# vfrantc/Bayesian-Enhancement-Model

Hardware: AMD Instinct MI355X
Metric: images/sec (whole node) CG_UNet N=8 Bayesian eval @256x256 (higher is better)
Workload: dtype f32

## Files before the change

### bayesian-enhancement-model_amd/csrc/conv.hip

```cpp
#include "bem_common.h"

namespace {

constexpr int RB = 4;

__device__ __forceinline__ void dw_block(const float* __restrict__ plane, int H, int W, int y0, int x0, bool vec,
                                         const float* __restrict__ w9, float (&acc)[RB][4]) {
    float wk[9];
#pragma unroll
    for (int i = 0; i < 9; ++i) wk[i] = w9[i];
#pragma unroll
    for (int ry = -1; ry <= RB; ++ry) {
        const int yy = y0 + ry;
        if (yy < 0 || yy >= H) continue;
        const float* r = plane + (int64_t)yy * W;
        float v[6];
        v[0] = x0 > 0 ? r[x0 - 1] : 0.f;
        if (vec) {
            const float4 c = *reinterpret_cast<const float4*>(r + x0);
            v[1] = c.x; v[2] = c.y; v[3] = c.z; v[4] = c.w;
        } else {
#pragma unroll
            for (int i = 0; i < 4; ++i) v[1 + i] = (x0 + i < W) ? r[x0 + i] : 0.f;
        }
        v[5] = (x0 + 4 < W) ? r[x0 + 4] : 0.f;
#pragma unroll
        for (int oy = 0; oy < RB; ++oy) {
            const int dy = ry - oy;
            if (dy < -1 || dy > 1) continue;
            const float w0 = wk[(dy + 1) * 3], w1 = wk[(dy + 1) * 3 + 1], w2 = wk[(dy + 1) * 3 + 2];
#pragma unroll
            for (int j = 0; j < 4; ++j) acc[oy][j] = fmaf(w0, v[j], fmaf(w1, v[j + 1], fmaf(w2, v[j + 2], acc[oy][j])));
        }
    }
}

__global__ __launch_bounds__(256) void dwconv3x3_kernel(const float* __restrict__ x, const float* __restrict__ w,
                                                        int64_t w_bs, const float* __restrict__ bias, int64_t b_bs,
                                                        float* __restrict__ out, int Cout, int H, int W, int mode) {
    const int W4 = (W + 3) >> 2, HB = (H + RB - 1) / RB;
    const int i = blockIdx.x * blockDim.x + threadIdx.x;
    if (i >= HB * W4) return;
    const int yb = i / W4, y0 = yb * RB, x0 = (i - yb * W4) * 4;
    const int c = blockIdx.y, b = blockIdx.z;
    const int Cin = (mode == 2) ? 2 * Cout : Cout;
    const int64_t HW = (int64_t)H * W;
    const bool vec = (W & 3) == 0;
    const float* wb = w + (int64_t)b * w_bs;
    const float* bb = bias ? bias + (int64_t)b * b_bs : nullptr;
    float a0[RB][4];
#pragma unroll
    for (int r = 0; r < RB; ++r)
#pragma unroll
        for (int j = 0; j < 4; ++j) a0[r][j] = 0.f;
    const float* pl = x + ((int64_t)b * Cin + c) * HW;
    dw_block(pl, H, W, y0, x0, vec, wb + (int64_t)c * 9, a0);
    const float b0 = bb ? bb[c] : 0.f;
    float a1[RB][4];
    float b1 = 0.f;
    if (mode == 2) {
#pragma unroll
        for (int r = 0; r < RB; ++r)
#pragma unroll
            for (int j = 0; j < 4; ++j) a1[r][j] = 0.f;
        dw_block(x + ((int64_t)b * Cin + c + Cout) * HW, H, W, y0, x0, vec, wb + (int64_t)(c + Cout) * 9, a1);
        b1 = bb ? bb[c + Cout] : 0.f;
    }
#pragma unroll
    for (int r = 0; r < RB; ++r) {
        const int y = y0 + r;
        if (y >= H) break;
        float o[4];
#pragma unroll
        for (int j = 0; j < 4; ++j) {
            const float v = a0[r][j] + b0;
            if (mode == 2) o[j] = bem_gelu(v) * (a1[r][j] + b1);
            else if (mode == 1) o[j] = bem_silu(v);
            else if (mode == 3) o[j] = ((x0 + j < W) ? pl[(int64_t)y * W + x0 + j] : 0.f) + fmaxf(v, 0.f);
            else o[j] = v;
        }
        float* op = out + ((int64_t)b * Cout + c) * HW + (int64_t)y * W + x0;
        if (vec) {
            *reinterpret_cast<float4*>(op) = make_float4(o[0], o[1], o[2], o[3]);
        } else {
#pragma unroll
            for (int j = 0; j < 4; ++j)
                if (x0 + j < W) op[j] = o[j];
        }
    }
}

__device__ __forceinline__ float dpp_from_prev_lane(float v) {
    return __builtin_bit_cast(float, __builtin_amdgcn_update_dpp(0, __builtin_bit_cast(int, v), 0x138, 0xf, 0xf, false));
}
__device__ __forceinline__ float dpp_from_next_lane(float v) {
    return __builtin_bit_cast(float, __builtin_amdgcn_update_dpp(0, __builtin_bit_cast(int, v), 0x130, 0xf, 0xf, false));
}

template <bool DPPHALO>
__device__ __forceinline__ void dw_block_fast(const float* __restrict__ plane, int H, int W, int y0, int x0,
                                              const float* __restrict__ w9, float (&acc)[RB][4]) {
    float4 c[RB + 2];
    float hl[RB + 2], hr[RB + 2];
#pragma unroll
    for (int ry = -1; ry <= RB; ++ry) {
        const int yy = min(max(y0 + ry, 0), H - 1);
        const float* r = plane + (int64_t)yy * W;
        c[ry + 1] = *reinterpret_cast<const float4*>(r + x0);
        if (!DPPHALO) {
            hl[ry + 1] = r[max(x0 - 1, 0)];
            hr[ry + 1] = r[min(x0 + 4, W - 1)];
        }
    }
    float wk[9];
#pragma unroll
    for (int i = 0; i < 9; ++i) wk[i] = w9[i];
    const float mt = y0 > 0 ? 1.f : 0.f, mb = y0 + RB < H ? 1.f : 0.f;
    const float ml = x0 > 0 ? 1.f : 0.f, mr = x0 + 4 < W ? 1.f : 0.f;
#pragma unroll
    for (int ry = -1; ry <= RB; ++ry) {
        float4 q = c[ry + 1];
        if (ry == -1) { q.x *= mt; q.y *= mt; q.z *= mt; q.w *= mt; }
        if (ry == RB) { q.x *= mb; q.y *= mb; q.z *= mb; q.w *= mb; }
        const float v[6] = {(DPPHALO ? dpp_from_prev_lane(q.w) : hl[ry + 1] * ((ry == -1) ? mt : (ry == RB) ? mb : 1.f)) * ml, q.x, q.y, q.z, q.w,
                            (DPPHALO ? dpp_from_next_lane(q.x) : hr[ry + 1] * ((ry == -1) ? mt : (ry == RB) ? mb : 1.f)) * mr};
#pragma unroll
        for (int oy = 0; oy < RB; ++oy) {
            const int dy = ry - oy;
            if (dy < -1 || dy > 1) continue;
            const float w0 = wk[(dy + 1) * 3], w1 = wk[(dy + 1) * 3 + 1], w2 = wk[(dy + 1) * 3 + 2];
#pragma unroll
            for (int j = 0; j < 4; ++j) acc[oy][j] = fmaf(w0, v[j], fmaf(w1, v[j + 1], fmaf(w2, v[j + 2], acc[oy][j])));
        }
    }
}

template <int MODE, bool DPPHALO>
__global__ __launch_bounds__(256) void dwconv3x3_fast_kernel(const float* __restrict__ x, const float* __restrict__ w,
                                                             int64_t w_bs, const float* __restrict__ bias, int64_t b_bs,
                                                             float* __restrict__ out, int Cout, int H, int W) {
    const int W4 = W >> 2, HB = H / RB;
    const int i = blockIdx.x * blockDim.x + threadIdx.x;
    if (i >= HB * W4) return;
    const int yb = i / W4, y0 = yb * RB, x0 = (i - yb * W4) * 4;
    const int c = blockIdx.y, b = blockIdx.z;
    const int Cin = (MODE == 2) ? 2 * Cout : Cout;
    const int64_t HW = (int64_t)H * W;
    const float* wb = w + (int64_t)b * w_bs;
    const float* bb = bias ? bias + (int64_t)b * b_bs : wb;
    const float bm = bias ? 1.f : 0.f;
    const float b0 = bb[bias ? c : 0] * bm;
    const float b1 = (MODE == 2) ? bb[bias ? c + Cout : 0] * bm : 0.f;
    const float* pl = x + ((int64_t)b * Cin + c) * HW;
    float a0[RB][4], a1[RB][4];
#pragma unroll
    for (int r = 0; r < RB; ++r)
#pragma unroll
        for (int j = 0; j < 4; ++j) a0[r][j] = a1[r][j] = 0.f;
    dw_block_fast<DPPHALO>(pl, H, W, y0, x0, wb + (int64_t)c * 9, a0);
    if (MODE == 2) dw_block_fast<DPPHALO>(x + ((int64_t)b * Cin + c + Cout) * HW, H, W, y0, x0, wb + (int64_t)(c + Cout) * 9, a1);
    float4 self[RB];
    if (MODE == 3) {
#pragma unroll
        for (int r = 0; r < RB; ++r) self[r] = *reinterpret_cast<const float4*>(pl + (int64_t)(y0 + r) * W + x0);
    }
#pragma unroll
    for (int r = 0; r < RB; ++r) {
        float o[4];
        const float sv[4] = {MODE == 3 ? self[r].x : 0.f, MODE == 3 ? self[r].y : 0.f, MODE == 3 ? self[r].z : 0.f, MODE == 3 ? self[r].w : 0.f};
#pragma unroll
        for (int j = 0; j < 4; ++j) {
            const float v = a0[r][j] + b0;
            if (MODE == 2) o[j] = bem_gelu_fast(v) * (a1[r][j] + b1);
            else if (MODE == 1) o[j] = bem_silu(v);
            else if (MODE == 3) o[j] = sv[j] + fmaxf(v, 0.f);
            else o[j] = v;
        }
        *reinterpret_cast<float4*>(out + ((int64_t)b * Cout + c) * HW + (int64_t)(y0 + r) * W + x0) = make_float4(o[0], o[1], o[2], o[3]);
    }
}

constexpr int TH = 8, TW = 32, COB = 16, CIB = 8;

template <int KH, int KW, int S>
__global__ __launch_bounds__(256) void conv2d_kernel(const float* __restrict__ x, int64_t x_bs,
                                                     const float* __restrict__ w, const float* __restrict__ bias,
                                                     const float* __restrict__ res1, const float* __restrict__ res2,
                                                     float* __restrict__ out, int Cin, int H, int W, int Cout,
                                                     int Ho, int Wo, int pad, int relu, int tilesX, int res1_rep) {
    constexpr int PH = (TH - 1) * S + KH, PW = (TW - 1) * S + KW;
    constexpr int PWP = PW + 1;
    __shared__ float patch[CIB][PH][PWP];
    __shared__ __attribute__((aligned(16))) float wl[CIB][KH * KW][COB];
    const int tile = blockIdx.x;
    const int ty0 = (tile / tilesX) * TH, tx0 = (tile % tilesX) * TW;
    const int co0 = blockIdx.y * COB;
    const int b = blockIdx.z;
    const int tx = threadIdx.x & 31, ty = threadIdx.x >> 5;
    const int oy = ty0 + ty, ox = tx0 + tx;
    const int iy0 = ty0 * S - pad, ix0 = tx0 * S - pad;
    const float* xb = x + (int64_t)b * x_bs;
    float acc[COB];
#pragma unroll
    for (int i = 0; i < COB; ++i) acc[i] = 0.f;
    for (int ci0 = 0; ci0 < Cin; ci0 += CIB) {
        __syncthreads();
        for (int i = threadIdx.x; i < CIB * PH * PW; i += 256) {
            const int cc = i / (PH * PW), rem = i - cc * (PH * PW);
            const int py = rem / PW, px = rem - py * PW;
            const int ci = ci0 + cc, iy = iy0 + py, ix = ix0 + px;
            float v = 0.f;
            if (ci < Cin && iy >= 0 && iy < H && ix >= 0 && ix < W) v = xb[((int64_t)ci * H + iy) * W + ix];
            patch[cc][py][px] = v;
        }
        for (int i = threadIdx.x; i < CIB * KH * KW * COB; i += 256) {
            const int o = i % COB, t = (i / COB) % (KH * KW), cc = i / (COB * KH * KW);
            const int ci = ci0 + cc, co = co0 + o;
            wl[cc][t][o] = (ci < Cin && co < Cout) ? w[(((int64_t)co * Cin + ci) * KH * KW) + t] : 0.f;
        }
        __syncthreads();
#pragma unroll 2
        for (int cc = 0; cc < CIB; ++cc) {
#pragma unroll
            for (int ky = 0; ky < KH; ++ky) {
#pragma unroll
                for (int kx = 0; kx < KW; ++kx) {
                    const float v = patch[cc][ty * S + ky][tx * S + kx];
                    const float4* wq = reinterpret_cast<const float4*>(&wl[cc][ky * KW + kx][0]);
#pragma unroll
                    for (int q = 0; q < COB / 4; ++q) {
                        const float4 ww = wq[q];
                        acc[4 * q] = fmaf(ww.x, v, acc[4 * q]);
                        acc[4 * q + 1] = fmaf(ww.y, v, acc[4 * q + 1]);
                        acc[4 * q + 2] = fmaf(ww.z, v, acc[4 * q + 2]);
                        acc[4 * q + 3] = fmaf(ww.w, v, acc[4 * q + 3]);
                    }
                }
            }
        }
    }
    if (oy >= Ho || ox >= Wo) return;
#pragma unroll
    for (int o = 0; o < COB; ++o) {
        const int co = co0 + o;
        if (co >= Cout) break;
        float v = acc[o] + (bias ? bias[co] : 0.f);
        if (relu) v = fmaxf(v, 0.f);
        const int64_t idx = (((int64_t)b * Cout + co) * Ho + oy) * Wo + ox;
        if (res1) v += res1[(((int64_t)(b / res1_rep) * Cout + co) * Ho + oy) * Wo + ox];
        if (res2) v += res2[idx];
        out[idx] = v;
    }
}


typedef float f32x16 __attribute__((ext_vector_type(16)));

template <int KH, int KW, int PH, int PWP>
__device__ __forceinline__ constexpr int patch_off(int k) {
    return (k / (KH * KW)) * PH * PWP + ((k % (KH * KW)) / KW) * PWP + (k % (KH * KW)) % KW;
}

template <int MTW>
__device__ __forceinline__ void conv_mfma_epilogue(f32x16 (&acc)[MTW][2], const float* __restrict__ Wp, const float* __restrict__ bias,
                                                   const float* __restrict__ res1, const float* __restrict__ res2,
                                                   float* __restrict__ out, int b, int b1, int Cout, int Ho, int Wo, int ty0, int tx0,
                                                   int wave, int half, int j, int relu) {
    const int ox = tx0 + j, oxc = min(ox, Wo - 1);
    const float* bp = bias ? bias : Wp;
    const float* p1 = res1 ? res1 : Wp;
    const float* p2 = res2 ? res2 : Wp;
    const float bmk = bias ? 1.f : 0.f, m1 = res1 ? 1.f : 0.f, m2 = res2 ? 1.f : 0.f;
    const int64_t k0 = bias ? -1 : 0, k1 = res1 ? -1 : 0, k2 = res2 ? -1 : 0;
    const float lo = relu ? 0.f : -3.402823466e38f;
    const int64_t b1off = (int64_t)(b1 - b) * Cout * Ho * Wo;
#pragma unroll
    for (int t = 0; t < 2; ++t) {
        const int oy = ty0 + 2 * wave + t, oyc = min(oy, Ho - 1);
        const bool pix = oy < Ho && ox < Wo;
#pragma unroll
        for (int m = 0; m < MTW; ++m) {
            constexpr int RG = 8;
#pragma unroll
            for (int r0 = 0; r0 < 16; r0 += RG) {
                float r1[RG], r2[RG], bv[RG];
#pragma unroll
                for (int q = 0; q < RG; ++q) {
                    const int r = r0 + q;
                    const int co = min(m * 32 + (r & 3) + 8 * (r >> 2) + 4 * half, Cout - 1);
                    const int64_t idx = (((int64_t)b * Cout + co) * Ho + oyc) * Wo + oxc;
                    bv[q] = bp[co & k0] * bmk;
                    r1[q] = p1[(idx + b1off) & k1] * m1;
                    r2[q] = p2[idx & k2] * m2;
                }
#pragma unroll
                for (int q = 0; q < RG; ++q) {
                    const int r = r0 + q;
                    const int co = m * 32 + (r & 3) + 8 * (r >> 2) + 4 * half;
                    if (pix && co < Cout)
                        out[(((int64_t)b * Cout + co) * Ho + oy) * Wo + ox] = fmaxf(acc[m][t][r] + bv[q], lo) + r1[q] + r2[q];
                }
            }
        }
    }
}

template <int KH, int KW, int S, int MTW>
__global__ __launch_bounds__(256, MTW == 1 ? 4 : MTW == 2 ? 3 : MTW == 3 ? 2 : 1) void conv2d_mfma_kernel(const float* __restrict__ x, int64_t x_bs,
                                                          const float* __restrict__ Wp, const float* __restrict__ bias,
                                                          const float* __restrict__ res1, const float* __restrict__ res2,
                                                          float* __restrict__ out, int Cin, int H, int W, int Cout,
                                                          int Ho, int Wo, int pad, int relu, int tilesX, int KS, int res1_rep) {
    constexpr int KK = KH * KW;
    constexpr int KC = CIB * KK;
    constexpr int PH = (TH - 1) * S + KH, PW = (TW - 1) * S + KW, PWP = PW + 1;
    __shared__ float patch[CIB * PH * PWP];
    const int lane = threadIdx.x & 63, wave = threadIdx.x >> 6, half = lane >> 5, j = lane & 31;
    const int tile = blockIdx.x, b = blockIdx.y;
    const int ty0 = (tile / tilesX) * TH, tx0 = (tile % tilesX) * TW;
    const int iy0 = ty0 * S - pad, ix0 = tx0 * S - pad;
    const float* xb = x + (int64_t)b * x_bs;
    f32x16 acc[MTW][2];
#pragma unroll
    for (int m = 0; m < MTW; ++m)
#pragma unroll
        for (int t = 0; t < 2; ++t)
#pragma unroll
            for (int r = 0; r < 16; ++r) acc[m][t][r] = 0.f;
    const float* wl = Wp + lane;
    const int64_t mts = (int64_t)KS * 64;
    const int rowoff0 = (2 * wave) * S * PWP + j * S, rowoff1 = rowoff0 + S * PWP;
// ... 37 lines not shown
            for (int u = 0; u < PB; ++u)
                an[m][u] = wl[m * mts + (int64_t)min(sg0 + u, KS - 1) * 64] * ((sg0 + u < KS) ? 1.f : 0.f);
        for (int s0 = 0; s0 < NS; s0 += PB) {
            float ac[MTW][PB];
#pragma unroll
            for (int m = 0; m < MTW; ++m)
#pragma unroll
                for (int u = 0; u < PB; ++u) {
                    ac[m][u] = an[m][u];
                    const int sn = sg0 + s0 + PB + u;
                    an[m][u] = wl[m * mts + (int64_t)min(sn, KS - 1) * 64] * ((s0 + PB + u < NS && sn < KS) ? 1.f : 0.f);
                }
#pragma unroll
            for (int u = 0; u < PB; ++u) {
                const int k = 2 * (s0 + u) + half, kc = k / KK, kt = k - kc * KK;
                const int o = kc * PH * PWP + (kt / KW) * PWP + (kt % KW);
                const float v0 = patch[o + rowoff0], v1 = patch[o + rowoff1];
#pragma unroll
                for (int m = 0; m < MTW; ++m) {
                    acc[m][0] = __builtin_amdgcn_mfma_f32_32x32x2f32(ac[m][u], v0, acc[m][0], 0, 0, 0);
                    acc[m][1] = __builtin_amdgcn_mfma_f32_32x32x2f32(ac[m][u], v1, acc[m][1], 0, 0, 0);
                }
            }
        }
    }
    conv_mfma_epilogue<MTW>(acc, Wp, bias, res1, res2, out, b, b / res1_rep, Cout, Ho, Wo, ty0, tx0, wave, half, j, relu);
}

template <int KH, int KW, int S, int MTW>
__global__ __launch_bounds__(256, MTW == 1 ? 3 : 2) void conv2d_mfma_pipe_kernel(const float* __restrict__ x, int64_t x_bs,
                                                               const float* __restrict__ Wp, const float* __restrict__ bias,
                                                               const float* __restrict__ res1, const float* __restrict__ res2,
                                                               float* __restrict__ out, int Cin, int H, int W, int Cout,
                                                               int Ho, int Wo, int pad, int relu, int tilesX, int KS, int res1_rep) {
    constexpr int KK = KH * KW;
    constexpr int KC = CIB * KK;
    constexpr int NS = KC / 2;
    constexpr int PH = (TH - 1) * S + KH, PW = (TW - 1) * S + KW, PWP = PW + 1;
    constexpr int PSZ = CIB * PH * PWP;
    constexpr int TOT = CIB * PH * PW;
    constexpr int NU = (TOT + 255) / 256;
    constexpr int WSZ = NS * 64;
    static_assert(WSZ % 256 == 0, "weight slice must split evenly over the workgroup");
    constexpr int NWU = WSZ / 256;
    __shared__ float patch[2][PSZ + 1];
    __shared__ float wsm[2][MTW][WSZ];
    const int lane = threadIdx.x & 63, wave = threadIdx.x >> 6, half = lane >> 5, j = lane & 31;
    const int tile = blockIdx.x, b = blockIdx.y;
    const int ty0 = (tile / tilesX) * TH, tx0 = (tile % tilesX) * TW;
    const int iy0 = ty0 * S - pad, ix0 = tx0 * S - pad;
    const float* xb = x + (int64_t)b * x_bs;
    const int HW = H * W;
    int goff[NU], lofc[NU];
    float gm[NU];
#pragma unroll
    for (int u = 0; u < NU; ++u) {
        const int i = u * 256 + threadIdx.x;
        const int cc = i / (PH * PW), rem = i - cc * (PH * PW);
        const int py = rem / PW, px = rem - py * PW;
        const int iy = iy0 + py, ix = ix0 + px;
        const bool in = i < TOT && iy >= 0 && iy < H && ix >= 0 && ix < W;
        goff[u] = in ? iy * W + ix : 0;
        gm[u] = in ? 1.f : 0.f;
        lofc[u] = (i < TOT ? cc * PH * PWP + py * PWP + px : PSZ) | (min(cc, CIB - 1) << 20);
    }
    f32x16 acc[MTW][2];
#pragma unroll
    for (int m = 0; m < MTW; ++m)
#pragma unroll
        for (int t = 0; t < 2; ++t)
#pragma unroll
            for (int r = 0; r < 16; ++r) acc[m][t][r] = 0.f;
    const int64_t mts = (int64_t)KS * 64;
    const int wtot = KS * 64;
    const int rowoff0 = (2 * wave) * S * PWP + j * S, rowoff1 = rowoff0 + S * PWP;
    float v[NU], wv[MTW][NWU];
    auto fetch = [&](int ci0) {
#pragma unroll
        for (int u = 0; u < NU; ++u) {
            const float* p = xb + (int64_t)min(ci0 + (lofc[u] >> 20), Cin - 1) * HW + goff[u];
            asm volatile("global_load_dword %0, %1, off" : "=v"(v[u]) : "v"(p));
        }
        const int wbase = ((ci0 * KK) >> 1) * 64;
#pragma unroll
        for (int m = 0; m < MTW; ++m)
#pragma unroll
            for (int u = 0; u < NWU; ++u) {
                const float* p = Wp + m * mts + min(wbase + u * 256 + (int)threadIdx.x, wtot - 1);
                asm volatile("global_load_dword %0, %1, off" : "=v"(wv[m][u]) : "v"(p));
            }
    };
    auto arrive = [&]() {
        static_assert(NU == 11 && NWU == 9 && MTW <= 2, "operand lists below are written for the 3x3 stride-1 chunk");
        asm volatile("s_waitcnt vmcnt(0)"
                     : "+v"(v[0]), "+v"(v[1]), "+v"(v[2]), "+v"(v[3]), "+v"(v[4]), "+v"(v[5]), "+v"(v[6]), "+v"(v[7]), "+v"(v[8]),
                       "+v"(v[9]), "+v"(v[10]));
#pragma unroll
        for (int m = 0; m < MTW; ++m)
            asm volatile("" : "+v"(wv[m][0]), "+v"(wv[m][1]), "+v"(wv[m][2]), "+v"(wv[m][3]), "+v"(wv[m][4]), "+v"(wv[m][5]),
                              "+v"(wv[m][6]), "+v"(wv[m][7]), "+v"(wv[m][8]));
    };
    auto stash = [&](int bufi, int ci0) {
        const int wbase = ((ci0 * KK) >> 1) * 64;
#pragma unroll
        for (int u = 0; u < NU; ++u) patch[bufi][lofc[u] & 0xfffff] = v[u] * (ci0 + (lofc[u] >> 20) < Cin ? gm[u] : 0.f);
#pragma unroll
        for (int m = 0; m < MTW; ++m)
#pragma unroll
            for (int u = 0; u < NWU; ++u)
                wsm[bufi][m][u * 256 + threadIdx.x] = wv[m][u] * (wbase + u * 256 + (int)threadIdx.x < wtot ? 1.f : 0.f);
    };
    fetch(0);
    arrive();
    stash(0, 0);
    __syncthreads();
    int buf = 0;
    for (int ci0 = 0; ci0 < Cin; ci0 += CIB) {
        fetch(ci0 + CIB);
        __builtin_amdgcn_sched_barrier(0);
        const float* pb = patch[buf];
#pragma unroll
        for (int s = 0; s < NS; ++s) {
            const int o = half ? patch_off<KH, KW, PH, PWP>(2 * s + 1) : patch_off<KH, KW, PH, PWP>(2 * s);
            const float v0 = pb[o + rowoff0], v1 = pb[o + rowoff1];
#pragma unroll
            for (int m = 0; m < MTW; ++m) {
                const float a = wsm[buf][m][s * 64 + lane];
                acc[m][0] = __builtin_amdgcn_mfma_f32_32x32x2f32(a, v0, acc[m][0], 0, 0, 0);
                acc[m][1] = __builtin_amdgcn_mfma_f32_32x32x2f32(a, v1, acc[m][1], 0, 0, 0);
            }
        }
        __builtin_amdgcn_sched_barrier(0);
        arrive();
        stash(buf ^ 1, ci0 + CIB);
        __syncthreads();
        buf ^= 1;
    }
    conv_mfma_epilogue<MTW>(acc, Wp, bias, res1, res2, out, b, b / res1_rep, Cout, Ho, Wo, ty0, tx0, wave, half, j, relu);
}

}

extern "C" int bem_dwconv3x3_f32(const float* x, const float* w, int64_t w_bstride, const float* bias,
                                 int64_t bias_bstride, float* out, int B, int Cout, int H, int W, int mode,
                                 void* stream) {
    BEM_REQUIRE(x && w && out, "dwconv3x3: null tensor");
    BEM_REQUIRE(B >= 0 && B <= 65535 && Cout > 0 && Cout <= 65535 && H > 0 && W > 0, "dwconv3x3: bad shape");
    BEM_REQUIRE(mode >= 0 && mode <= 3, "dwconv3x3: mode %d", mode);
    if (B == 0) return BEM_OK;
    dim3 grid(cdiv(cdiv(H, RB) * ((W + 3) / 4), 256), Cout, B);
    hipStream_t s = (hipStream_t)stream;
    const bool fast = W % 4 == 0 && H % RB == 0 && (((uintptr_t)x | (uintptr_t)out) & 15) == 0;
    const bool dpp = fast && 64 % (W / 4) == 0;
#define BEM_DW(MODE) do { if (dpp) dwconv3x3_fast_kernel<MODE, true><<<grid, 256, 0, s>>>(x, w, w_bstride, bias, bias_bstride, out, Cout, H, W); \
                          else dwconv3x3_fast_kernel<MODE, false><<<grid, 256, 0, s>>>(x, w, w_bstride, bias, bias_bstride, out, Cout, H, W); } while (0)
    if (!fast) dwconv3x3_kernel<<<grid, 256, 0, s>>>(x, w, w_bstride, bias, bias_bstride, out, Cout, H, W, mode);
    else if (mode == 0) BEM_DW(0);
    else if (mode == 1) BEM_DW(1);
    else if (mode == 2) BEM_DW(2);
    else BEM_DW(3);
#undef BEM_DW
    return bem_check_launch("dwconv3x3");
}

extern "C" int bem_conv2d_f32(const float* x, int64_t x_bstride, const float* w, const float* bias,
                              const float* res1, const float* res2, float* out, int B, int Cin, int H, int W,
                              int Cout, int KH, int KW, int stride, int pad, int relu, int res1_rep, void* stream) {
    BEM_REQUIRE(x && w && out && res1_rep >= 1, "conv2d: null tensor or res1_rep < 1");
    BEM_REQUIRE(B >= 0 && B <= 65535 && Cin > 0 && Cout > 0 && H > 0 && W > 0, "conv2d: bad shape");
    const int Ho = (H + 2 * pad - KH) / stride + 1, Wo = (W + 2 * pad - KW) / stride + 1;
    BEM_REQUIRE(Ho > 0 && Wo > 0, "conv2d: empty output");
    if (B == 0) return BEM_OK;
    const int tilesX = cdiv(Wo, TW), tilesY = cdiv(Ho, TH);
    dim3 grid(tilesX * tilesY, cdiv(Cout, COB), B);
    hipStream_t s = (hipStream_t)stream;
    if (KH == 3 && KW == 3 && stride == 1)
        conv2d_kernel<3, 3, 1><<<grid, 256, 0, s>>>(x, x_bstride, w, bias, res1, res2, out, Cin, H, W, Cout, Ho, Wo, pad, relu, tilesX, res1_rep);
    else if (KH == 4 && KW == 4 && stride == 2)
        conv2d_kernel<4, 4, 2><<<grid, 256, 0, s>>>(x, x_bstride, w, bias, res1, res2, out, Cin, H, W, Cout, Ho, Wo, pad, relu, tilesX, res1_rep);
    else
        BEM_REQUIRE(false, "conv2d: unsupported kernel %dx%d stride %d (have 3x3 s1, 4x4 s2)", KH, KW, stride);
    return bem_check_launch("conv2d");
}

extern "C" int bem_conv2d_mfma_f32(const float* x, int64_t x_bstride, const float* Wp, const float* bias,
                                   const float* res1, const float* res2, float* out, int B, int Cin, int H, int W,
                                   int Cout, int KH, int KW, int stride, int pad, int relu, int res1_rep, void* stream) {
    BEM_REQUIRE(x && Wp && out && res1_rep >= 1, "conv2d_mfma: null tensor or res1_rep < 1");
    BEM_REQUIRE(B >= 0 && B <= 65535 && Cin > 0 && Cout > 0 && Cout <= 160 && H > 0 && W > 0, "conv2d_mfma: bad shape (Cout <= 160)");
    const int Ho = (H + 2 * pad - KH) / stride + 1, Wo = (W + 2 * pad - KW) / stride + 1;
    BEM_REQUIRE(Ho > 0 && Wo > 0, "conv2d_mfma: empty output");
    if (B == 0) return BEM_OK;
    const int tilesX = cdiv(Wo, TW), tilesY = cdiv(Ho, TH);
    const int KS = cdiv(Cin * KH * KW, 2), MT = cdiv(Cout, 32);
    dim3 grid(tilesX * tilesY, B);
    hipStream_t s = (hipStream_t)stream;
#define BEM_CONV_LAUNCH(KH_, KW_, S_, MTW_) \
    conv2d_mfma_kernel<KH_, KW_, S_, MTW_><<<grid, 256, 0, s>>>(x, x_bstride, Wp, bias, res1, res2, out, Cin, H, W, Cout, Ho, Wo, pad, relu, tilesX, KS, res1_rep)
    if (KH == 3 && KW == 3 && stride == 1) {
        if (MT <= 2) {
            if (MT == 1) conv2d_mfma_pipe_kernel<3, 3, 1, 1><<<grid, 256, 0, s>>>(x, x_bstride, Wp, bias, res1, res2, out, Cin, H, W, Cout, Ho, Wo, pad, relu, tilesX, KS, res1_rep);
            else conv2d_mfma_pipe_kernel<3, 3, 1, 2><<<grid, 256, 0, s>>>(x, x_bstride, Wp, bias, res1, res2, out, Cin, H, W, Cout, Ho, Wo, pad, relu, tilesX, KS, res1_rep);
        }
        else if (MT == 3) BEM_CONV_LAUNCH(3, 3, 1, 3);
        else BEM_CONV_LAUNCH(3, 3, 1, 5);
    } else if (KH == 4 && KW == 4 && stride == 2) {
        if (MT == 1) BEM_CONV_LAUNCH(4, 4, 2, 1);
        else if (MT == 2) BEM_CONV_LAUNCH(4, 4, 2, 2);
        else if (MT == 3) BEM_CONV_LAUNCH(4, 4, 2, 3);
        else BEM_CONV_LAUNCH(4, 4, 2, 5);
    } else {
        BEM_REQUIRE(false, "conv2d_mfma: unsupported kernel %dx%d stride %d (have 3x3 s1, 4x4 s2)", KH, KW, stride);
    }
#undef BEM_CONV_LAUNCH
    return bem_check_launch("conv2d_mfma");
}
```

### bayesian-enhancement-model_amd/csrc/pw_gemm_x6.hip

```cpp
#include "bem_common.h"
#include "x6_common.h"
#include <algorithm>

namespace {


struct PwX {
    const float* x1; const float* x2; int C1; int C2; int in_mode;
    const float* ln_w; const float* ln_b; float ln_eps;
    const u32x4* Wp; int64_t w_bstride;
    const float* bias; int64_t bias_bstride;
    const float* res; const float* prelu; int act;
    float* out; int out_mode; int Win;
    int M; int K; int L; int KB; int MT;
    int mtpb;
};


template <int NSUB, bool SUM, bool VEC>
__device__ __forceinline__ void ldx(const PwX& k, int b, int ch, int pc, const bool (&keep)[NSUB], float (&o)[NSUB]) {
    const int chc = min(ch, k.K - 1);
    const bool first = chc < k.C1;
    const float* r1 = k.x1 + ((int64_t)b * k.C1 + (first ? chc : 0)) * k.L;
    const float* r2 = k.x2 + ((int64_t)b * k.C2 + (first ? 0 : chc - k.C1)) * k.L;
// ... 353 lines not shown
            for (int e = 0; e < 8; ++e) {
                const float g = valu_copy(s_ln[16 * kb + 8 * kh + e]), be = valu_copy(s_ln[16 * KBM + 16 * kb + 8 * kh + e]);
                xr[kb][e][0] = (xr[kb][e][0] - mean) * rstd * g + be;
            }
    }
    u32x4 xl[KBM][3];
#pragma unroll
    for (int kb = 0; kb < KBM; ++kb) {
        float v[8];
#pragma unroll
        for (int e = 0; e < 8; ++e) v[e] = xr[kb][e][0];
        split8(v, xl[kb][0], xl[kb][1], xl[kb][2]);
    }
    int buf = 0;
    for (int mt0 = mt_lo; mt0 < mt_hi; ++mt0, buf ^= 1) {
        asm volatile("s_waitcnt vmcnt(0)" ::: "memory");
        __syncthreads();
        if (mt0 + 1 < mt_hi) dma(mt0 + 1, buf ^ 1);
        f32x16 acc[1][1], alo;
        float4 bq[1][4];
        x6_load_bias<1>(k, b, mt0, kh, bq);
        acc[0][0] = alo = zero16();
        const u32x4* wl = &Ws[buf][lane];
        u32x4 wn[3] = {wl[0], wl[64], wl[128]};
#pragma unroll
        for (int kb = 0; kb < KBM; ++kb) {
            const u32x4 wc[3] = {wn[0], wn[1], wn[2]};
            if (kb + 1 < KBM) {
                wn[0] = wl[((kb + 1) * 3 + 0) * 64]; wn[1] = wl[((kb + 1) * 3 + 1) * 64]; wn[2] = wl[((kb + 1) * 3 + 2) * 64];
            }
            __builtin_amdgcn_sched_barrier(0);
            mac6(wc, xl[kb], acc[0][0], alo);
            __builtin_amdgcn_sched_barrier(0);
        }
        acc[0][0] += alo;
        x6_epilogue<1, 1, VEC>(k, b, mt0, p, keep, kh, s_bias, bq, acc);
    }
}

constexpr int BEM_X6_MAXK_LN = 1024;
template <int MTW, int NSUB, bool SUM, bool VEC, bool LN>
__global__ __launch_bounds__(256, 2) void pw_x6_stream_kernel(PwX k) {
    const int lane = threadIdx.x & 63, wave = threadIdx.x >> 6, kh = lane >> 5, n = lane & 31;
    const int b = blockIdx.z, mt0 = blockIdx.y * MTW;
    const int p0 = (xcd_tile(blockIdx.x, gridDim.x) * 4 + wave) * (32 * NSUB);
    __shared__ __attribute__((aligned(16))) float s_bias[BEM_X6_MAXM];
    __shared__ float s_ln[LN ? 2 * BEM_X6_MAXK_LN : 2];
    stage_bias(k, b, s_bias);
    if (LN) {
        for (int i = threadIdx.x; i < k.KB * 16; i += 256) {
            s_ln[i] = i < k.K ? k.ln_w[i] : 0.f;
            s_ln[BEM_X6_MAXK_LN + i] = i < k.K ? k.ln_b[i] : 0.f;
        }
    }
    __syncthreads();
    if (p0 >= k.L) return;
    const int p = p0 + NSUB * n;
    bool keep[NSUB];
#pragma unroll
    for (int t = 0; t < NSUB; ++t) keep[t] = p + t < k.L;
    const int pc = VEC ? (keep[0] ? p : 0) : p;
    auto load_x = [&](int kb, float (&dst)[8][NSUB]) {
#pragma unroll
        for (int e = 0; e < 8; ++e) ldx<NSUB, SUM, VEC>(k, b, 16 * kb + 8 * kh + e, pc, keep, dst[e]);
    };
    float mean[NSUB], rstd[NSUB];
    if (LN) {
        const float inv = 1.f / (float)k.K;
        float s[NSUB];
#pragma unroll
        for (int t = 0; t < NSUB; ++t) s[t] = 0.f;
        for (int kb = 0; kb < k.KB; ++kb) {
            float v[8][NSUB];
            load_x(kb, v);
#pragma unroll
            for (int e = 0; e < 8; ++e)
#pragma unroll
                for (int t = 0; t < NSUB; ++t) s[t] += v[e][t];
        }
#pragma unroll
        for (int t = 0; t < NSUB; ++t) { s[t] += __shfl_xor(s[t], 32, 64); mean[t] = s[t] * inv; }
        float q[NSUB];
#pragma unroll
        for (int t = 0; t < NSUB; ++t) q[t] = 0.f;
        for (int kb = 0; kb < k.KB; ++kb) {
            float v[8][NSUB];
            load_x(kb, v);
#pragma unroll
            for (int e = 0; e < 8; ++e) {
                const float mk = (16 * kb + 8 * kh + e < k.K) ? 1.f : 0.f;
#pragma unroll
                for (int t = 0; t < NSUB; ++t) { const float d = (v[e][t] - mean[t]) * mk; q[t] = fmaf(d, d, q[t]); }
            }
        }
#pragma unroll
        for (int t = 0; t < NSUB; ++t) { q[t] += __shfl_xor(q[t], 32, 64); rstd[t] = 1.f / sqrtf(q[t] * inv + k.ln_eps); }
    }
    f32x16 acc[MTW][NSUB], alo[MTW][NSUB];
#pragma unroll
for (int m = 0; m < MTW; ++m)
#pragma unroll
        for (int t = 0; t < NSUB; ++t)
#pragma unroll
            for (int r = 0; r < 16; ++r) acc[m][t][r] = alo[m][t][r] = 0.f;
    const u32x4* wbase = k.Wp + (int64_t)b * k.w_bstride + lane;
    const int64_t mt_stride = (int64_t)k.KB * 3 * 64;
    auto load_w = [&](int kb, u32x4 (&dst)[MTW][3]) {
#pragma unroll
        for (int m = 0; m < MTW; ++m) {
            const bool ok = kb < k.KB && mt0 + m < k.MT;
            const u32x4* wp = wbase + (int64_t)(mt0 + m < k.MT ? mt0 + m : 0) * mt_stride + (int64_t)min(kb, k.KB - 1) * 3 * 64;
            load_w3_masked(wp, ok ? 0xffffffffu : 0u, dst[m]);
        }
    };
    float xn[8][NSUB], xn2[8][NSUB];
    u32x4 wn[MTW][3];
    load_x(0, xn);
    load_x(1, xn2);
    load_w(0, wn);
    for (int kb = 0; kb < k.KB; ++kb) {
        u32x4 xl[NSUB][3], wc[MTW][3];
#pragma unroll
        for (int t = 0; t < NSUB; ++t) {
            float v[8];
#pragma unroll
            for (int e = 0; e < 8; ++e) {
                v[e] = xn[e][t];
                if (LN) v[e] = (v[e] - mean[t]) * rstd[t] * valu_copy(s_ln[16 * kb + 8 * kh + e]) + valu_copy(s_ln[BEM_X6_MAXK_LN + 16 * kb + 8 * kh + e]);
            }
            split8(v, xl[t][0], xl[t][1], xl[t][2]);
        }
#pragma unroll
        for (int m = 0; m < MTW; ++m)
#pragma unroll
            for (int li = 0; li < 3; ++li) wc[m][li] = wn[m][li];
#pragma unroll
        for (int e = 0; e < 8; ++e)
#pragma unroll
            for (int t = 0; t < NSUB; ++t) xn[e][t] = xn2[e][t];
        load_x(kb + 2, xn2);
        load_w(kb + 1, wn);
#pragma unroll
        for (int m = 0; m < MTW; ++m)
#pragma unroll
            for (int t = 0; t < NSUB; ++t) mac6(wc[m], xl[t], acc[m][t], alo[m][t]);
    }
#pragma unroll
    for (int m = 0; m < MTW; ++m)
#pragma unroll
        for (int t = 0; t < NSUB; ++t) acc[m][t] += alo[m][t];
    float4 bq[MTW][4];
    x6_load_bias<MTW>(k, b, mt0, kh, bq);
    x6_epilogue<MTW, NSUB, VEC>(k, b, mt0, p, keep, kh, s_bias, bq, acc);
}

}

extern "C" int bem_pw_gemm_x6_f32(const bem_pw_args* a, void* stream) {
    BEM_REQUIRE(a, "pw_gemm_x6: null args");
    BEM_REQUIRE(a->x1 && a->Wp && a->out, "pw_gemm_x6: null tensor");
    BEM_REQUIRE(a->B >= 0 && a->B <= 65535 && a->M > 0 && a->M <= BEM_X6_MAXM && a->K > 0 && a->L >= 0, "pw_gemm_x6: bad shape B=%d M=%d K=%d L=%d", a->B, a->M, a->K, a->L);
    BEM_REQUIRE(a->in_mode >= 0 && a->in_mode <= 2, "pw_gemm_x6: in_mode %d", a->in_mode);
    if (a->in_mode == 0) BEM_REQUIRE(a->K == a->C1, "pw_gemm_x6: K %d != C1 %d", a->K, a->C1);
    if (a->in_mode == 1) BEM_REQUIRE(a->x2 && a->K == a->C1 && a->C1 == a->C2, "pw_gemm_x6: sum mode needs x2 and K == C1 == C2");
    if (a->in_mode == 2) BEM_REQUIRE(a->x2 && a->K == a->C1 + a->C2, "pw_gemm_x6: cat mode needs x2 and K == C1 + C2");
    BEM_REQUIRE((a->ln_w == nullptr) == (a->ln_b == nullptr), "pw_gemm_x6: ln_w / ln_b must both be set or both NULL");
    BEM_REQUIRE(a->act == 0 || (a->act == 1 && a->prelu), "pw_gemm_x6: act %d", a->act);
    BEM_REQUIRE(a->out_mode == 0 || (a->out_mode == 1 && a->M % 4 == 0 && a->Win > 0 && a->L % a->Win == 0 && !a->res),
                "pw_gemm_x6: out_mode %d constraints", a->out_mode);
    BEM_REQUIRE(((uintptr_t)a->Wp & 15) == 0 && a->w_bstride % 4 == 0, "pw_gemm_x6: packed weights must be 16-byte aligned");
    BEM_REQUIRE((int64_t)a->M * a->L < (1ll << 30), "pw_gemm_x6: M * L = %lld exceeds the 32-bit lane offsets of the epilogue", (long long)a->M * a->L);
    const bool ln = a->ln_w != nullptr;
    BEM_REQUIRE(!ln || a->K <= BEM_X6_MAXK_LN, "pw_gemm_x6: LayerNorm prologue supports K <= %d (got %d)", BEM_X6_MAXK_LN, a->K);
    if (a->B == 0 || a->L == 0) return BEM_OK;
    PwX k;
    k.x1 = a->x1; k.x2 = a->x2 ? a->x2 : a->x1; k.C1 = a->C1; k.C2 = a->x2 ? a->C2 : a->C1; k.in_mode = a->in_mode;
    k.ln_w = a->ln_w; k.ln_b = a->ln_b; k.ln_eps = a->ln_eps;
    k.Wp = reinterpret_cast<const u32x4*>(a->Wp); k.w_bstride = a->w_bstride / 4; k.bias = a->bias; k.bias_bstride = a->bias_bstride;
    k.res = a->res; k.prelu = a->prelu; k.act = a->act; k.out = a->out; k.out_mode = a->out_mode; k.Win = a->Win;
    k.M = a->M; k.K = a->K; k.L = a->L; k.KB = cdiv(a->K, 16); k.MT = cdiv(a->M, 32); k.mtpb = k.MT;
    hipStream_t s = (hipStream_t)stream;
    const bool sum = a->in_mode == 1;
    const bool al = (((uintptr_t)a->x1 | (uintptr_t)(a->x2 ? a->x2 : a->x1) | (uintptr_t)a->out | (uintptr_t)(a->res ? a->res : a->out)) & 7) == 0;
    const bool vec = a->L % 2 == 0 && al;
#define BEM_X6_RES(KBM, NSUB, MTW)                                                                       \
    do {                                                                                                 \
        dim3 grid(cdiv(a->L, 128 * NSUB), 1, a->B);                                                      \
                    \
        const int64_t wv = (int64_t)a->B * cdiv(a->L, 32 * NSUB);                                        \
        const int groups = cdiv(k.MT, MTW);                                                              \
        const int ny = wv >= 2048 ? 1 : (int)std::min<int64_t>(groups, cdiv64(2048, wv));                \
        k.mtpb = cdiv(groups, ny) * MTW;                                                                 \
        grid.y = cdiv(k.MT, k.mtpb);                                                                     \
        if (NSUB == 2 && vec && !sum) pw_x6_res_kernel<KBM, NSUB, MTW, false, true><<<grid, 256, 0, s>>>(k);   \
        else if (NSUB == 2 && vec) pw_x6_res_kernel<KBM, NSUB, MTW, true, true><<<grid, 256, 0, s>>>(k);       \
        else if (!sum) pw_x6_res_kernel<KBM, NSUB, MTW, false, false><<<grid, 256, 0, s>>>(k);                 \
        else pw_x6_res_kernel<KBM, NSUB, MTW, true, false><<<grid, 256, 0, s>>>(k);                            \
        return bem_check_launch("pw_x6_res");                                                            \
    } while (0)
    if (k.KB <= 3) BEM_X6_RES(3, 2, 1);
    if (ln && k.KB <= 5) BEM_X6_RES(5, 2, 1);
    if (ln && k.KB == 10 && k.K == 160 && k.MT >= 8 && (int64_t)a->B * cdiv(a->L, 32) >= 2048) {
        dim3 grid(cdiv(a->L, 128), 1, a->B);
        k.mtpb = k.MT;
        if (!sum) pw_x6_res_lds_kernel<10, false, false><<<grid, 256, 0, s>>>(k);
        else pw_x6_res_lds_kernel<10, true, false><<<grid, 256, 0, s>>>(k);
        return bem_check_launch("pw_x6_res_lds");
    }
    if (ln && k.KB <= 10) { if (k.MT == 1) BEM_X6_RES(10, 1, 1); else BEM_X6_RES(10, 1, 2); }
#undef BEM_X6_RES
    {
        const int mtw = k.MT == 1 ? 1 : 2;
        dim3 grid(cdiv(a->L, 256), cdiv(k.MT, mtw), a->B);
#define BEM_X6_STREAM(MTW, LN)                                                                \
    do {                                                                                      \
        if (vec && !sum) pw_x6_stream_kernel<MTW, 2, false, true, LN><<<grid, 256, 0, s>>>(k);   \
        else if (vec) pw_x6_stream_kernel<MTW, 2, true, true, LN><<<grid, 256, 0, s>>>(k);       \
        else if (!sum) pw_x6_stream_kernel<MTW, 2, false, false, LN><<<grid, 256, 0, s>>>(k);    \
        else pw_x6_stream_kernel<MTW, 2, true, false, LN><<<grid, 256, 0, s>>>(k);               \
    } while (0)
        if (ln) { if (mtw == 1) BEM_X6_STREAM(1, true); else BEM_X6_STREAM(2, true); }
        else { if (mtw == 1) BEM_X6_STREAM(1, false); else BEM_X6_STREAM(2, false); }
#undef BEM_X6_STREAM
    }
    return bem_check_launch("pw_x6_stream");
}
```

Measured before the change: 327.7.

## Pack multiple channels per block for tiny dwconv and split-K small pointwise GEMM

For depthwise 3x3 convs whose spatial plane needs at most 16 threads, several channels are now packed into one 256-thread block instead of launching a mostly idle block per channel, with masking for out-of-range channels. A new split-K pointwise GEMM kernel handles tiny spatial sizes (L <= 128). It spreads the K reduction across waves, combines the partials through LDS, and supports an optional LayerNorm prologue. Both target the low-resolution bottleneck levels of the UNet, where occupancy is poor. The cost is extra synchronisation and LDS traffic, plus added kernel variants.

```diff
diff --git a/bayesian-enhancement-model_amd/csrc/conv.hip b/bayesian-enhancement-model_amd/csrc/conv.hip
--- a/bayesian-enhancement-model_amd/csrc/conv.hip
+++ b/bayesian-enhancement-model_amd/csrc/conv.hip
@@ -97,7 +97,7 @@
     return __builtin_bit_cast(float, __builtin_amdgcn_update_dpp(0, __builtin_bit_cast(int, v), 0x130, 0xf, 0xf, false));
 }
 
-template <bool DPPHALO>
+template <bool DPPHALO, bool VW = false>
 __device__ __forceinline__ void dw_block_fast(const float* __restrict__ plane, int H, int W, int y0, int x0,
                                               const float* __restrict__ w9, float (&acc)[RB][4]) {
     float4 c[RB + 2];
@@ -114,7 +114,7 @@
     }
     float wk[9];
 #pragma unroll
-    for (int i = 0; i < 9; ++i) wk[i] = w9[i];
+    for (int i = 0; i < 9; ++i) wk[i] = VW ? valu_copy(w9[i]) : w9[i];
     const float mt = y0 > 0 ? 1.f : 0.f, mb = y0 + RB < H ? 1.f : 0.f;
     const float ml = x0 > 0 ? 1.f : 0.f, mr = x0 + 4 < W ? 1.f : 0.f;
 #pragma unroll
@@ -122,8 +122,12 @@
         float4 q = c[ry + 1];
         if (ry == -1) { q.x *= mt; q.y *= mt; q.z *= mt; q.w *= mt; }
         if (ry == RB) { q.x *= mb; q.y *= mb; q.z *= mb; q.w *= mb; }
-        const float v[6] = {(DPPHALO ? dpp_from_prev_lane(q.w) : hl[ry + 1] * ((ry == -1) ? mt : (ry == RB) ? mb : 1.f)) * ml, q.x, q.y, q.z, q.w,
-                            (DPPHALO ? dpp_from_next_lane(q.x) : hr[ry + 1] * ((ry == -1) ? mt : (ry == RB) ? mb : 1.f)) * mr};
+        float v[6] = {(DPPHALO ? dpp_from_prev_lane(q.w) : hl[ry + 1] * ((ry == -1) ? mt : (ry == RB) ? mb : 1.f)) * ml, q.x, q.y, q.z, q.w,
+                      (DPPHALO ? dpp_from_next_lane(q.x) : hr[ry + 1] * ((ry == -1) ? mt : (ry == RB) ? mb : 1.f)) * mr};
+        if (VW && DPPHALO) {
+            v[0] = x0 > 0 ? v[0] : 0.f;
+            v[5] = x0 + 4 < W ? v[5] : 0.f;
+        }
 #pragma unroll
         for (int oy = 0; oy < RB; ++oy) {
             const int dy = ry - oy;
@@ -135,30 +139,39 @@
     }
 }
 
-template <int MODE, bool DPPHALO>
+template <int MODE, bool DPPHALO, bool GROUP>
 __global__ __launch_bounds__(256) void dwconv3x3_fast_kernel(const float* __restrict__ x, const float* __restrict__ w,
                                                              int64_t w_bs, const float* __restrict__ bias, int64_t b_bs,
                                                              float* __restrict__ out, int Cout, int H, int W) {
     const int W4 = W >> 2, HB = H / RB;
-    const int i = blockIdx.x * blockDim.x + threadIdx.x;
-    if (i >= HB * W4) return;
+    int i = blockIdx.x * blockDim.x + threadIdx.x;
+    int c = blockIdx.y;
+    bool live = true;
+    if (GROUP) {
+        const int per = HB * W4, cg = 256 / per, ci = (int)threadIdx.x / per;
+        i = (int)threadIdx.x - ci * per;
+        c = blockIdx.y * cg + ci;
+        live = ci < cg && c < Cout;
+        c = min(c, Cout - 1);
+    } else if (i >= HB * W4) return;
     const int yb = i / W4, y0 = yb * RB, x0 = (i - yb * W4) * 4;
-    const int c = blockIdx.y, b = blockIdx.z;
+    const int b = blockIdx.z;
     const int Cin = (MODE == 2) ? 2 * Cout : Cout;
     const int64_t HW = (int64_t)H * W;
     const float* wb = w + (int64_t)b * w_bs;
     const float* bb = bias ? bias + (int64_t)b * b_bs : wb;
     const float bm = bias ? 1.f : 0.f;
-    const float b0 = bb[bias ? c : 0] * bm;
-    const float b1 = (MODE == 2) ? bb[bias ? c + Cout : 0] * bm : 0.f;
+    float b0 = bb[bias ? c : 0] * bm;
+    float b1 = (MODE == 2) ? bb[bias ? c + Cout : 0] * bm : 0.f;
+    if (GROUP) { b0 = valu_copy(b0); b1 = valu_copy(b1); }
     const float* pl = x + ((int64_t)b * Cin + c) * HW;
     float a0[RB][4], a1[RB][4];
 #pragma unroll
     for (int r = 0; r < RB; ++r)
 #pragma unroll
         for (int j = 0; j < 4; ++j) a0[r][j] = a1[r][j] = 0.f;
-    dw_block_fast<DPPHALO>(pl, H, W, y0, x0, wb + (int64_t)c * 9, a0);
-    if (MODE == 2) dw_block_fast<DPPHALO>(x + ((int64_t)b * Cin + c + Cout) * HW, H, W, y0, x0, wb + (int64_t)(c + Cout) * 9, a1);
+    dw_block_fast<DPPHALO, GROUP>(pl, H, W, y0, x0, wb + (int64_t)c * 9, a0);
+    if (MODE == 2) dw_block_fast<DPPHALO, GROUP>(x + ((int64_t)b * Cin + c + Cout) * HW, H, W, y0, x0, wb + (int64_t)(c + Cout) * 9, a1);
     float4 self[RB];
     if (MODE == 3) {
 #pragma unroll
@@ -176,7 +189,7 @@
             else if (MODE == 3) o[j] = sv[j] + fmaxf(v, 0.f);
             else o[j] = v;
         }
-        *reinterpret_cast<float4*>(out + ((int64_t)b * Cout + c) * HW + (int64_t)(y0 + r) * W + x0) = make_float4(o[0], o[1], o[2], o[3]);
+        if (!GROUP || live) *reinterpret_cast<float4*>(out + ((int64_t)b * Cout + c) * HW + (int64_t)(y0 + r) * W + x0) = make_float4(o[0], o[1], o[2], o[3]);
     }
 }
 
@@ -520,8 +533,13 @@
     hipStream_t s = (hipStream_t)stream;
     const bool fast = W % 4 == 0 && H % RB == 0 && (((uintptr_t)x | (uintptr_t)out) & 15) == 0;
     const bool dpp = fast && 64 % (W / 4) == 0;
-#define BEM_DW(MODE) do { if (dpp) dwconv3x3_fast_kernel<MODE, true><<<grid, 256, 0, s>>>(x, w, w_bstride, bias, bias_bstride, out, Cout, H, W); \
-                          else dwconv3x3_fast_kernel<MODE, false><<<grid, 256, 0, s>>>(x, w, w_bstride, bias, bias_bstride, out, Cout, H, W); } while (0)
+    const int per = (H / RB) * (W / 4);
+    const bool group = fast && per <= 16;
+    if (group) grid = dim3(1, cdiv(Cout, 256 / per), B);
+#define BEM_DW(MODE) do { if (group && dpp) dwconv3x3_fast_kernel<MODE, true, true><<<grid, 256, 0, s>>>(x, w, w_bstride, bias, bias_bstride, out, Cout, H, W); \
+                          else if (group) dwconv3x3_fast_kernel<MODE, false, true><<<grid, 256, 0, s>>>(x, w, w_bstride, bias, bias_bstride, out, Cout, H, W); \
+                          else if (dpp) dwconv3x3_fast_kernel<MODE, true, false><<<grid, 256, 0, s>>>(x, w, w_bstride, bias, bias_bstride, out, Cout, H, W); \
+                          else dwconv3x3_fast_kernel<MODE, false, false><<<grid, 256, 0, s>>>(x, w, w_bstride, bias, bias_bstride, out, Cout, H, W); } while (0)
     if (!fast) dwconv3x3_kernel<<<grid, 256, 0, s>>>(x, w, w_bstride, bias, bias_bstride, out, Cout, H, W, mode);
     else if (mode == 0) BEM_DW(0);
     else if (mode == 1) BEM_DW(1);
diff --git a/bayesian-enhancement-model_amd/csrc/pw_gemm_x6.hip b/bayesian-enhancement-model_amd/csrc/pw_gemm_x6.hip
--- a/bayesian-enhancement-model_amd/csrc/pw_gemm_x6.hip
+++ b/bayesian-enhancement-model_amd/csrc/pw_gemm_x6.hip
@@ -529,6 +529,150 @@
     float4 bq[MTW][4];
     x6_load_bias<MTW>(k, b, mt0, kh, bq);
     x6_epilogue<MTW, NSUB, VEC>(k, b, mt0, p, keep, kh, s_bias, bq, acc);
+}
+
+constexpr int BEM_X6_SMALL_D = 3;
+template <int KS, int NSUB, bool SUM, bool VEC, bool LN>
+__global__ __launch_bounds__(256, 2) void pw_x6_small_kernel(PwX k) {
+    constexpr int PW = 4 / KS, D = BEM_X6_SMALL_D, MAXK = 16 * 4 * D;
+    const int lane = threadIdx.x & 63, wave = __builtin_amdgcn_readfirstlane(threadIdx.x >> 6), kh = lane >> 5, n = lane & 31;
+    const int pg = wave / KS, ks = wave % KS;
+    const int b = blockIdx.z, mt0 = blockIdx.y;
+    __shared__ __attribute__((aligned(16))) float s_bias[BEM_X6_MAXM];
+    __shared__ float s_ln[LN ? 2 * MAXK : 2];
+    __shared__ float s_stat[LN ? 2 * 4 * NSUB * 64 : 2];
+    __shared__ float s_part[PW * (KS - 1) * NSUB * 16 * 64];
+    stage_bias(k, b, s_bias);
+    if (LN) {
+        for (int i = threadIdx.x; i < k.KB * 16; i += 256) {
+            s_ln[i] = i < k.K ? k.ln_w[i] : 0.f;
+            s_ln[MAXK + i] = i < k.K ? k.ln_b[i] : 0.f;
+        }
+    }
+    __syncthreads();
+    const int p = pg * (32 * NSUB) + NSUB * n;
+    bool keep[NSUB];
+#pragma unroll
+    for (int t = 0; t < NSUB; ++t) keep[t] = p + t < k.L;
+    const int pc = VEC ? (keep[0] ? p : 0) : p;
+    const int q = (k.KB + KS - 1) / KS, kb0 = ks * q, kb1 = min(k.KB, kb0 + q);
+    const u32x4* wbase = k.Wp + (int64_t)b * k.w_bstride + (int64_t)mt0 * k.KB * 3 * 64 + lane;
+    f32x16 acc[1][NSUB], alo[NSUB];
+#pragma unroll
+    for (int t = 0; t < NSUB; ++t) acc[0][t] = alo[t] = zero16();
+    int kc = kb0;
+#pragma nounroll
+    do {
+        u32x4 wv[D][3];
+        float xv[D][8][NSUB];
+#pragma unroll
+        for (int d = 0; d < D; ++d) {
+            load_w3_masked(wbase + (int64_t)min(kc + d, k.KB - 1) * 3 * 64, kc + d < kb1 ? 0xffffffffu : 0u, wv[d]);
+#pragma unroll
+            for (int e = 0; e < 8; ++e) ldx<NSUB, SUM, VEC>(k, b, 16 * (kc + d) + 8 * kh + e, pc, keep, xv[d][e]);
+        }
+        float mean[NSUB], rstd[NSUB];
+        if (LN) {
+            const float inv = 1.f / (float)k.K;
+            float* st = s_stat + lane;
+#pragma unroll
+            for (int t = 0; t < NSUB; ++t) {
+                float sm = 0.f;
+#pragma unroll
+                for (int d = 0; d < D; ++d)
+                    if (kc + d < kb1) {
+#pragma unroll
+                        for (int e = 0; e < 8; ++e) sm += xv[d][e][t];
+                    }
+                sm += __shfl_xor(sm, 32, 64);
+                st[((pg * KS + ks) * NSUB + t) * 64] = sm;
+            }
+            __syncthreads();
+#pragma unroll
+            for (int t = 0; t < NSUB; ++t) {
+                float sm = 0.f;
+#pragma unroll
+                for (int j = 0; j < KS; ++j) sm += valu_copy(st[((pg * KS + j) * NSUB + t) * 64]);
+                mean[t] = sm * inv;
+                float sq = 0.f;
+#pragma unroll
+                for (int d = 0; d < D; ++d)
+                    if (kc + d < kb1) {
+#pragma unroll
+                        for (int e = 0; e < 8; ++e) {
+                            const float dv = (16 * (kc + d) + 8 * kh + e < k.K) ? xv[d][e][t] - mean[t] : 0.f;
+                            sq = fmaf(dv, dv, sq);
+                        }
+                    }
+                sq += __shfl_xor(sq, 32, 64);
+                st[(4 * NSUB + (pg * KS + ks) * NSUB + t) * 64] = sq;
+            }
+            __syncthreads();
+#pragma unroll
+            for (int t = 0; t < NSUB; ++t) {
+                float sq = 0.f;
+#pragma unroll
+                for (int j = 0; j < KS; ++j) sq += valu_copy(st[(4 * NSUB + (pg * KS + j) * NSUB + t) * 64]);
+                rstd[t] = 1.f / sqrtf(sq * inv + k.ln_eps);
+            }
+        }
+#pragma unroll
+        for (int d = 0; d < D; ++d) {
+            if (kc + d < kb1) {
+                u32x4 xl[NSUB][3];
+#pragma unroll
+                for (int t = 0; t < NSUB; ++t) {
+                    float v[8];
+#pragma unroll
+                    for (int e = 0; e < 8; ++e) {
+                        v[e] = xv[d][e][t];
+                        const int ch = min(16 * (kc + d) + 8 * kh + e, MAXK - 1);
+                        if (LN) v[e] = (v[e] - mean[t]) * rstd[t] * valu_copy(s_ln[ch]) + valu_copy(s_ln[MAXK + ch]);
+                    }
+                    split8(v, xl[t][0], xl[t][1], xl[t][2]);
+                }
+#pragma unroll
+                for (int t = 0; t < NSUB; ++t) mac6(wv[d], xl[t], acc[0][t], alo[t]);
+            }
+        }
+        kc += D;
+    } while (kc < kb1);
+#pragma unroll
+    for (int t = 0; t < NSUB; ++t) acc[0][t] += alo[t];
+    float4 bq[1][4];
+    x6_load_bias<1>(k, b, mt0, kh, bq);
+    float* sp = s_part + (int64_t)(pg * (KS - 1) * NSUB) * 1024 + lane;
+    if (ks != 0) {
+#pragma unroll
+        for (int t = 0; t < NSUB; ++t)
+#pragma unroll
+            for (int r = 0; r < 16; ++r) sp[(((ks - 1) * NSUB + t) * 16 + r) * 64] = acc[0][t][r];
+    }
+    __syncthreads();
+    if (ks != 0) return;
+#pragma unroll
+    for (int j = 1; j < KS; ++j)
+#pragma unroll
+        for (int t = 0; t < NSUB; ++t)
+#pragma unroll
+            for (int r = 0; r < 16; ++r) acc[0][t][r] += valu_copy(sp[(((j - 1) * NSUB + t) * 16 + r) * 64]);
+    x6_epilogue<1, NSUB, VEC>(k, b, mt0, p, keep, kh, s_bias, bq, acc);
+}
+
+template <int KS, int NSUB>
+void launch_small(const PwX& k, dim3 grid, hipStream_t s, bool sum, bool vec, bool ln) {
+#define BEM_X6_SMALL(SUM, VEC)                                                              \
+    do {                                                                                    \
+        if constexpr (NSUB == 1) {                                                          \
+            if (ln) { pw_x6_small_kernel<KS, NSUB, SUM, VEC, true><<<grid, 256, 0, s>>>(k); break; }   \
+        }                                                                                   \
+        pw_x6_small_kernel<KS, NSUB, SUM, VEC, false><<<grid, 256, 0, s>>>(k);              \
+    } while (0)
+    if (NSUB == 2 && vec && !sum) BEM_X6_SMALL(false, NSUB == 2);
+    else if (NSUB == 2 && vec) BEM_X6_SMALL(true, NSUB == 2);
+    else if (!sum) BEM_X6_SMALL(false, false);
+    else BEM_X6_SMALL(true, false);
+#undef BEM_X6_SMALL
 }
 
 }
@@ -563,7 +707,7 @@
 #define BEM_X6_RES(KBM, NSUB, MTW)                                                                       \
     do {                                                                                                 \
         dim3 grid(cdiv(a->L, 128 * NSUB), 1, a->B);                                                      \
-                    \
+                                   \
         const int64_t wv = (int64_t)a->B * cdiv(a->L, 32 * NSUB);                                        \
         const int groups = cdiv(k.MT, MTW);                                                              \
         const int ny = wv >= 2048 ? 1 : (int)std::min<int64_t>(groups, cdiv64(2048, wv));                \
@@ -575,6 +719,16 @@
         else pw_x6_res_kernel<KBM, NSUB, MTW, true, false><<<grid, 256, 0, s>>>(k);                            \
         return bem_check_launch("pw_x6_res");                                                            \
     } while (0)
+    if (a->L <= 128 && k.KB > 3) {
+        const int ks = a->L <= 64 ? 4 : 2;
+        if (!ln || (a->L <= 32 && cdiv(k.KB, ks) <= BEM_X6_SMALL_D)) {
+            const dim3 grid(1, k.MT, a->B);
+            if (a->L <= 32) launch_small<4, 1>(k, grid, s, sum, vec, ln);
+            else if (ks == 4) launch_small<4, 2>(k, grid, s, sum, vec, ln);
+            else launch_small<2, 2>(k, grid, s, sum, vec, ln);
+            return bem_check_launch("pw_x6_small");
+        }
+    }
     if (k.KB <= 3) BEM_X6_RES(3, 2, 1);
     if (ln && k.KB <= 5) BEM_X6_RES(5, 2, 1);
     if (ln && k.KB == 10 && k.K == 160 && k.MT >= 8 && (int64_t)a->B * cdiv(a->L, 32) >= 2048) {
```

New measurement: 336.8, median of 6. 2.8% higher.
